# undistro/trivy

Hardware: AMD Instinct MI355X
Metric: GB/s secret-scanned (whole node) at 1/2/4/8 MI355X; findings bit-exact vs CPU (higher is better)
Workload: dtype u8

## Files before the change

### trivy_amd/csrc/engine.hip

```cpp
#include <chrono>
#include <condition_variable>
#include <mutex>
#include <hip/hip_runtime.h>

#include <algorithm>
#include <cstdlib>
#include <cstdio>
#include <cstring>
#include <string>
#include <pthread.h>

#include <thread>
#include <type_traits>

#include "engine.h"
#include "fetch.h"
#include "fetch_host.h"
#include "fetch_windows.h"
#include "xform.h"
#include "filter.h"

namespace tsg {

namespace {

constexpr int kScanThreads = 1024;
constexpr int kScanWaves = kScanThreads / 64;

#define HIP_OK(x)                                                   \
  do {                                                              \
    hipError_t e_ = (x);                                            \
    if (e_ != hipSuccess) {                                         \
      err_ = std::string(#x) + ": " + hipGetErrorString(e_);        \
      return false;                                                 \
    }                                                               \
  } while (0)


constexpr uint32_t kK0Run = 16;
struct ClearParams {
  uint32_t* flags;
  uint32_t* kw;
  uint64_t n_kw;
  uint32_t* counters;
  uint32_t* fs_ctr;
  uint32_t* skip_info;
};
__device__ __forceinline__ void clear_words(uint32_t* p, uint64_t n, uint64_t tid, uint64_t nthr) {
  const uint64_t n4 = n / 4;
  for (uint64_t i = tid; i < n4; i += nthr) reinterpret_cast<uint4*>(p)[i] = make_uint4(0, 0, 0, 0);
  if (tid < n % 4) p[4 * n4 + tid] = 0;
}
__global__ __launch_bounds__(256) void chunk_map_kernel(const uint64_t* __restrict__ off, uint32_t n_files,
                                                        uint64_t n_chunks, uint32_t* __restrict__ chunk_file,
                                                        ClearParams Z) {
  {
    const uint64_t tid = uint64_t(blockIdx.x) * blockDim.x + threadIdx.x, nthr = uint64_t(gridDim.x) * blockDim.x;
    clear_words(Z.flags, n_files, tid, nthr);
    clear_words(Z.kw, Z.n_kw, tid, nthr);
    if (tid < 16) {
      Z.counters[tid] = 0;
      if (Z.fs_ctr) Z.fs_ctr[tid] = 0;
      if (Z.skip_info) Z.skip_info[tid] = 0;
    }
  }
  const uint64_t n_runs = (n_chunks + kK0Run - 1) / kK0Run;
  for (uint64_t r = uint64_t(blockIdx.x) * blockDim.x + threadIdx.x; r < n_runs;
       r += uint64_t(gridDim.x) * blockDim.x) {
    const uint64_t c0 = r * kK0Run;
    uint64_t x = c0 * kChunk;
    uint32_t lo = 0, hi = n_files;
    while (hi - lo > 1) {
      const uint32_t mid = (lo + hi) >> 1;
      if (off[mid] <= x) lo = mid;
      else hi = mid;
    }
    uint32_t v[kK0Run];
    uint64_t fe = off[lo + 1];
#pragma unroll
    for (uint32_t i = 0; i < kK0Run; i++) {
      x = (c0 + i) * kChunk;
      while (x >= fe && lo + 1 < n_files) fe = off[++lo + 1];
      v[i] = lo;
    }
    if (c0 + kK0Run <= n_chunks) {
      uint4* d = reinterpret_cast<uint4*>(chunk_file + c0);
#pragma unroll
      for (uint32_t q = 0; q < kK0Run / 4; q++) d[q] = make_uint4(v[4 * q], v[4 * q + 1], v[4 * q + 2], v[4 * q + 3]);
    } else {
      for (uint32_t i = 0; c0 + i < n_chunks; i++) chunk_file[c0 + i] = v[i];
    }
  }
}

__device__ __forceinline__ uint4 load16(const uint8_t* p) { return *reinterpret_cast<const uint4*>(p); }

__device__ __forceinline__ void wave_sync() {
  __builtin_amdgcn_fence(__ATOMIC_RELEASE, "wavefront");
  __builtin_amdgcn_wave_barrier();
  __builtin_amdgcn_fence(__ATOMIC_ACQUIRE, "wavefront");
}

constexpr int kFLane = 64;
constexpr int kFBlocks = kFLane / 16;
constexpr int kFTile = 64 * kFLane;
constexpr int kFFlushAt = 128;
constexpr int kFQueue = kFFlushAt + 64;
constexpr int kFChunks = kFTile / 1024;
#ifndef TSG_K1_NLTILES
#define TSG_K1_NLTILES 16
#endif
constexpr int kFNlTiles = TSG_K1_NLTILES;
#ifndef TSG_K1_WGS
#define TSG_K1_WGS 2
#endif
constexpr int kFWgPerCu = TSG_K1_WGS;
#ifndef TSG_K1_GROUPQ
#define TSG_K1_GROUPQ 1
#endif
constexpr uint32_t kFGroup = 8;
#ifndef TSG_K1_READAHEAD
#define TSG_K1_READAHEAD 4
#endif
constexpr uint32_t kFReadAhead = TSG_K1_READAHEAD;
constexpr int kFWindow = 6;
constexpr int kFWords = 4;
constexpr uint32_t kFireBits = 0xFFF00000u;
constexpr uint32_t kNlBits = 0x8888u;
static_assert(kChunk % kFLane == 0 && kChunk / kFLane <= 64, "a newline chunk must be whole lane chunks");
static_assert(kFChunks * kChunk == kFTile && kFChunks == 4, "a tile's newline counts are one u64");

constexpr uint32_t kSkRuns = 0, kSkKept = 1, kSkTailKept = 2, kSkFiles = 3, kSkBytes = 4 ,
                   kSkWaveRuns = 6, kSkTiles = 7;

constexpr uint32_t kRunWords = 8;
__host__ __device__ inline uint64_t KeepWords(uint64_t n_tiles) {
  return ((n_tiles + 63) / 64 + kRunWords - 1) / kRunWords * kRunWords;
}

__global__ __launch_bounds__(256) void tile_keep_kernel(const uint64_t* __restrict__ off, uint32_t n_files,
                                                        const uint32_t* __restrict__ chunk_file,
                                                        const uint8_t* __restrict__ skip, uint64_t n_bytes,
                                                        uint64_t n_tiles, uint64_t* __restrict__ keep_bits,
                                                        uint32_t* __restrict__ info) {
  const uint32_t lane = threadIdx.x & 63u;
  const uint64_t stride = uint64_t(gridDim.x) * blockDim.x;
  const uint64_t n_padded = KeepWords(n_tiles) * 64;
  for (uint64_t base = uint64_t(blockIdx.x) * blockDim.x + (threadIdx.x & ~63u); base < n_padded; base += stride) {
    const uint64_t t = base + lane;
    bool keep = false;
    if (t < n_tiles) {
      const uint64_t ts = t * kFTile, te = ts + kFTile < n_bytes ? ts + kFTile : n_bytes;
      uint32_t f = chunk_file[t * kFChunks];
      for (;;) {
        const uint64_t fb = off[f], fe = off[f + 1];
        if (fe > fb && !skip[f]) {
          keep = true;
          break;
        }
        if (fe >= te || f + 1 >= n_files) break;
        f++;
      }
    }
    const uint64_t m = __ballot(keep);
    if (lane == 0) keep_bits[base / 64] = m;
  }
  constexpr uint32_t kStatBlocks = 64;
  if (blockIdx.x >= kStatBlocks) return;
  const uint64_t fstride = uint64_t(gridDim.x < kStatBlocks ? gridDim.x : kStatBlocks) * blockDim.x;
  uint32_t nf = 0;
  uint64_t nb = 0;
  for (uint64_t f = uint64_t(blockIdx.x) * blockDim.x + threadIdx.x; f < n_files; f += fstride)
    if (skip[f]) {
      nf++;
      nb += off[f + 1] - off[f];
    }
#pragma unroll
  for (int x = 1; x < 64; x <<= 1) {
    nf += __shfl_xor(nf, x);
    nb += __shfl_xor(nb, x);
  }
  if (lane == 0 && nf) {
    atomicAdd(&info[kSkFiles], nf);
    atomicAdd(reinterpret_cast<unsigned long long*>(&info[kSkBytes]), static_cast<unsigned long long>(nb));
  }
}

constexpr int kRunThreads = 1024;
__global__ __launch_bounds__(kRunThreads) void tile_runs_kernel(const uint64_t* __restrict__ keep_bits,
                                                                uint64_t n_tiles, uint2* __restrict__ runs,
                                                                uint32_t* __restrict__ info) {
  __shared__ uint32_t s_k[kRunThreads / 64], s_r[kRunThreads / 64];
  const uint32_t tid = threadIdx.x, lane = tid & 63u, wv = tid >> 6;
  const uint64_t n_words = KeepWords(n_tiles);
  const uint64_t per = ((n_words / kRunWords + kRunThreads - 1) / kRunThreads) * kRunWords;
  const uint64_t w0 = per * tid < n_words ? per * tid : n_words;
  const uint64_t w1 = w0 + per < n_words ? w0 + per : n_words;
  const uint64_t carry0 = w0 > 0 && w0 < n_words ? keep_bits[w0 - 1] >> 63 : 0;
  auto load_group = [&](uint64_t w, uint64_t* b) {
    const uint4* g = reinterpret_cast<const uint4*>(keep_bits + w);
#pragma unroll
    for (uint32_t q = 0; q < kRunWords / 2; q++) {
      const uint4 v = g[q];
      b[2 * q] = uint64_t(v.x) | (uint64_t(v.y) << 32);
      b[2 * q + 1] = uint64_t(v.z) | (uint64_t(v.w) << 32);
    }
  };
  uint32_t kept = 0, starts = 0;
  uint64_t carry = carry0;
  for (uint64_t w = w0; w < w1; w += kRunWords) {
    uint64_t g[kRunWords];
    load_group(w, g);
#pragma unroll
    for (uint32_t q = 0; q < kRunWords; q++) {
      const uint64_t b = g[q];
      kept += uint32_t(__popcll(b));
      starts += uint32_t(__popcll(b & ~((b << 1) | carry)));
      carry = b >> 63;
    }
  }
  uint32_t ik = kept, ir = starts;
#pragma unroll
  for (int x = 1; x < 64; x <<= 1) {
    const uint32_t a = __shfl_up(ik, x), b = __shfl_up(ir, x);
    if (lane >= uint32_t(x)) {
      ik += a;
      ir += b;
    }
  }
  if (lane == 63) {
    s_k[wv] = ik;
    s_r[wv] = ir;
  }
  __syncthreads();
  uint32_t bk = 0, br = 0;
  for (uint32_t q = 0; q < wv; q++) {
    bk += s_k[q];
    br += s_r[q];
  }
  uint32_t k = bk + ik - kept, r = br + ir - starts;
  carry = carry0;
  for (uint64_t w = w0; w < w1; w += kRunWords) {
    uint64_t g[kRunWords];
    load_group(w, g);
#pragma unroll
    for (uint32_t q = 0; q < kRunWords; q++) {
      const uint64_t b = g[q];
      for (uint64_t s = b & ~((b << 1) | carry); s; s &= s - 1) {
        const uint32_t bit = uint32_t(__builtin_ctzll(s));
        runs[r++] = make_uint2(uint32_t((w + q) * 64 + bit), k + uint32_t(__popcll(b & ((uint64_t(1) << bit) - 1))));
      }
      k += uint32_t(__popcll(b));
      carry = b >> 63;
    }
  }
  if (tid == kRunThreads - 1) {
    runs[r] = make_uint2(uint32_t(n_tiles), k);
    info[kSkRuns] = r;
    info[kSkKept] = k;
    info[kSkTailKept] = n_tiles ? uint32_t((keep_bits[(n_tiles - 1) / 64] >> ((n_tiles - 1) & 63)) & 1) : 0u;
    info[kSkTiles] = uint32_t(n_tiles);
  }
}

struct FilterParams {
  const uint8_t* arena;
  uint64_t n_bytes;
  const uint2* runs;
  uint32_t* run_info;
  const uint32_t* reach;
  uint32_t diag_mode;
  uint16_t* nl;
  uint32_t* recs;
  uint32_t rec_cap;
  uint32_t* counters;
};

__device__ __forceinline__ uint4 reach_read(const uint8_t* sb, uint32_t w, uint32_t k, uint32_t laneoff) {
  return *reinterpret_cast<const uint4*>(sb + __builtin_amdgcn_perm(w, laneoff, 0x0C0C0000u | ((4u + k) << 8)));
}

__device__ __forceinline__ void reach_apply(const uint4& m, uint32_t* st) {
  asm("v_lshl_or_b32 %0, %1, 4, %2" : "=v"(st[0]) : "v"(st[0]), "v"(m.x));
  asm("v_lshl_or_b32 %0, %1, 4, %2" : "=v"(st[1]) : "v"(st[1]), "v"(m.y));
  asm("v_lshl_or_b32 %0, %1, 4, %2" : "=v"(st[2]) : "v"(st[2]), "v"(m.z));
  asm("v_lshl_or_b32 %0, %1, 4, %2" : "=v"(st[3]) : "v"(st[3]), "v"(m.w));
}

__device__ __forceinline__ uint32_t nl_count4(uint32_t w) {
  const uint32_t a = ((w ^ 0x0A0A0A0Au) & 0x7F7F7F7Fu) + 0x7F7F7F7Fu;
  return __popc(~(a | w) & 0x80808080u);
}

__device__ __forceinline__ uint32_t word_of(uint4 v, uint32_t i) {
  return i < 2 ? (i == 0 ? v.x : v.y) : (i == 2 ? v.z : v.w);
}

__device__ __forceinline__ void load_reach_lds(uint8_t* s_reach, const uint32_t* reach, uint32_t copies, int tid,
                                               int nthreads) {
  for (uint32_t i = tid; i < 256 * copies; i += nthreads) {
    const uint32_t b = i / copies;
    reinterpret_cast<uint4*>(s_reach)[i] = reinterpret_cast<const uint4*>(reach)[b];
  }
}

template <bool kRuns>
__global__ __launch_bounds__(kScanThreads, 8) void filter_kernel(FilterParams P) {
  __shared__ __attribute__((aligned(16))) uint8_t s_reach[65536];
  __shared__ uint32_t s_queue[kScanWaves * kFQueue];
  __shared__ uint64_t s_nl[kScanWaves * kFNlTiles];
  const int tid = threadIdx.x;
  load_reach_lds(s_reach, P.reach, 16, tid, blockDim.x);
  __syncthreads();
  const uint32_t lane = tid & 63;
  const uint32_t wave = __builtin_amdgcn_readfirstlane(uint32_t(tid) >> 6);
  const uint32_t laneoff = (lane & 15) * 16;
  uint32_t* Q = s_queue + wave * kFQueue;
  uint64_t* NL = s_nl + wave * kFNlTiles;
  uint32_t nl_slots = 0;
  uint32_t qn = 0;
  const uint64_t n_tiles = (P.n_bytes + kFTile - 1) / kFTile;
  const uint64_t n_waves = uint64_t(gridDim.x) * kScanWaves;
  const uint64_t wid = uint64_t(blockIdx.x) * kScanWaves + wave;
  const uint2* __restrict__ RUNS = kRuns ? P.runs : nullptr;
  auto uni = [](uint32_t v) { return uint32_t(__builtin_amdgcn_readfirstlane(v)); };
  const uint64_t n_kept = RUNS ? uint64_t(uni(P.run_info[kSkKept])) : n_tiles;
  const bool tail_kept = RUNS ? uni(P.run_info[kSkTailKept]) != 0 : true;
  const uint64_t per = n_kept / n_waves, extra = n_kept % n_waves;
  const uint64_t k_begin = wid * per + (wid < extra ? wid : extra);
  const uint64_t k_end = k_begin + per + (wid < extra ? 1 : 0);
  uint32_t run = 0;
  uint64_t run_k1 = n_kept;
  uint64_t t_begin = k_begin;
  uint32_t runs_walked = 1;
  if (RUNS && k_begin < k_end) {
    uint32_t lo = 0, hi = uni(P.run_info[kSkRuns]);
    while (hi - lo > 1) {
      const uint32_t mid = (lo + hi) >> 1;
      if (uni(RUNS[mid].y) <= k_begin) lo = mid;
      else hi = mid;
    }
    run = lo;
    const uint2 r0 = RUNS[lo];
    t_begin = uint64_t(uni(r0.x)) + (k_begin - uni(r0.y));
    run_k1 = uni(RUNS[lo + 1].y);
  }
  uint4 bufA[kFBlocks], bufB[kFBlocks];
  uint32_t pre_x = 0, pre_y = 0;
  auto load_pre = [&](uint64_t tt) {
    const uint2 pv = *reinterpret_cast<const uint2*>(P.arena + tt * kFTile - 8);
    pre_x = __builtin_amdgcn_readfirstlane(pv.x);
    pre_y = __builtin_amdgcn_readfirstlane(pv.y);
  };
  if (k_begin < k_end && t_begin > 0) load_pre(t_begin);
  auto next_tile = [&](uint64_t k1, uint64_t tcur, bool* nr) -> uint64_t {
    if (k1 < run_k1) {
      *nr = false;
      return tcur + 1;
    }
    run++;
    runs_walked++;
    run_k1 = uni(RUNS[run + 1].y);
    *nr = true;
    return uni(RUNS[run].x);
  };
  auto load_tile = [&](uint4* dst, uint64_t tt) {
    const uint64_t b0 = tt * kFTile + uint64_t(lane) * kFLane;
    const uint8_t* lp = P.arena + (b0 < P.n_bytes ? b0 : 0);
#pragma unroll
    for (int j = 0; j < kFBlocks; j++) dst[j] = load16(lp + 16 * j);
  };
  auto flush = [&]() {
    uint32_t base = 0;
    if (lane == 0) base = atomicAdd(&P.counters[7], qn);
    base = __builtin_amdgcn_readfirstlane(base);
    for (uint32_t i = lane; i < qn; i += 64) {
      if (base + i < P.rec_cap) P.recs[base + i] = Q[i];
      else P.counters[8] = 1;
    }
    qn = 0;
  };
#if TSG_K1_GROUPQ
  uint32_t fl_acc = 0;
  uint32_t grp_n = 0;
  uint64_t grp_t0 = 0;
  auto compact = [&]() {
    const uint32_t cnt = __popc(fl_acc);
    uint32_t incl = cnt;
    incl += uint32_t(__builtin_amdgcn_update_dpp(0, int(incl), 0x111, 0xF, 0xF, true));
    incl += uint32_t(__builtin_amdgcn_update_dpp(0, int(incl), 0x112, 0xF, 0xF, true));
    incl += uint32_t(__builtin_amdgcn_update_dpp(0, int(incl), 0x114, 0xF, 0xF, true));
    incl += uint32_t(__builtin_amdgcn_update_dpp(0, int(incl), 0x118, 0xF, 0xF, true));
    incl += uint32_t(__builtin_amdgcn_update_dpp(0, int(incl), 0x142, 0xA, 0xF, false));
    incl += uint32_t(__builtin_amdgcn_update_dpp(0, int(incl), 0x143, 0xC, 0xF, false));
    const uint32_t total = __builtin_amdgcn_readlane(incl, 63);
    if (total) {
      if (qn + total > kFQueue) flush();
      const uint32_t rec0 = __builtin_amdgcn_readfirstlane(uint32_t(grp_t0 * (kFTile / 16))) + lane * kFBlocks;
      uint32_t m = fl_acc;
      if (total <= kFQueue) {
        uint32_t at = qn + incl - cnt;
        while (m) {
          const uint32_t b = uint32_t(__builtin_ctz(m));
          m &= m - 1;
          Q[at++] = rec0 + ((b >> 2) << 8) + (b & 3u);
        }
        qn += total;
      } else {
        uint32_t base = 0;
        if (lane == 0) base = atomicAdd(&P.counters[7], total);
        uint32_t at = __builtin_amdgcn_readfirstlane(base) + incl - cnt;
        while (m) {
          const uint32_t b = uint32_t(__builtin_ctz(m));
          m &= m - 1;
          if (at < P.rec_cap) P.recs[at] = rec0 + ((b >> 2) << 8) + (b & 3u);
          else P.counters[8] = 1;
          at++;
        }
      }
    }
    fl_acc = 0;
    grp_n = 0;
  };
#endif
  auto flush_nl = [&](uint64_t t_last) {
    wave_sync();
    uint32_t l = lane;
    asm volatile("" : "+v"(l));
    if (l < nl_slots) {
      const uint64_t tt = t_last - uint64_t(nl_slots - 1 - l);
      reinterpret_cast<uint64_t*>(P.nl)[tt] = NL[l];
    }
    nl_slots = 0;
  };
  auto tile = [&](uint4* cur, uint64_t tt, auto tail_tag) {
    constexpr bool kTail = decltype(tail_tag)::value;
    if (kTail) {
      const uint64_t b0 = tt * kFTile + uint64_t(lane) * kFLane;
#pragma unroll
      for (int j = 0; j < kFBlocks; j++) {
        const uint64_t p = b0 + 16 * j;
        uint32_t wd[4] = {cur[j].x, cur[j].y, cur[j].z, cur[j].w};
#pragma unroll
        for (int q = 0; q < 4; q++) {
          const uint64_t wp = p + 4 * q;
          if (wp >= P.n_bytes) wd[q] = 0;
          else if (wp + 4 > P.n_bytes) wd[q] &= (1u << (8 * (P.n_bytes - wp))) - 1u;
        }
        cur[j] = make_uint4(wd[0], wd[1], wd[2], wd[3]);
      }
    }
    const uint32_t p0 = uint32_t(__builtin_amdgcn_update_dpp(int(pre_x), int(cur[kFBlocks - 1].z), 0x138, 0xF, 0xF,
                                                             false));
    const uint32_t p1 = uint32_t(__builtin_amdgcn_update_dpp(int(pre_y), int(cur[kFBlocks - 1].w), 0x138, 0xF, 0xF,
                                                             false));
    pre_x = __builtin_amdgcn_readlane(cur[kFBlocks - 1].z, 63);
    pre_y = __builtin_amdgcn_readlane(cur[kFBlocks - 1].w, 63);
    uint32_t flagged = 0, nl = 0;
    if (P.diag_mode < 2) {
      uint32_t st[kFWords] = {~0u, ~0u, ~0u, ~0u};
      reach_apply(reach_read(s_reach, p0, 3, laneoff), st);
#pragma unroll
      for (uint32_t k = 0; k < 4; k++) reach_apply(reach_read(s_reach, p1, k, laneoff), st);
#pragma unroll
      for (int j = 0; j < kFBlocks; j++) {
        const uint32_t wd[4] = {cur[j].x, cur[j].y, cur[j].z, cur[j].w};
        uint32_t acc = ~0u;
#pragma unroll
        for (uint32_t g = 0; g < 16; g += kFReadAhead) {
          uint4 m[kFReadAhead];
#pragma unroll
          for (uint32_t q = 0; q < kFReadAhead; q++)
            m[q] = reach_read(s_reach, wd[(g + q) >> 2], (g + q) & 3, laneoff);
#pragma unroll
          for (uint32_t q = 0; q < kFReadAhead; q++) {
            const uint32_t k = g + q;
            reach_apply(m[q], st);
            if (k % 3 == 2 || k == 15) acc &= st[0] & st[1] & st[2] & st[3];
            if (k % 4 == 3) nl += __popc(~st[3] & kNlBits);
          }
        }
        flagged |= uint32_t((acc | ~kFireBits) != ~0u) << j;
      }
    } else {
#pragma unroll
      for (int j = 0; j < kFBlocks; j++)
        nl += nl_count4(cur[j].x) + nl_count4(cur[j].y) + nl_count4(cur[j].z) + nl_count4(cur[j].w);
    }
    {
    nl += uint32_t(__builtin_amdgcn_update_dpp(0, int(nl), 0x111, 0xF, 0xF, true));
    nl += uint32_t(__builtin_amdgcn_update_dpp(0, int(nl), 0x112, 0xF, 0xF, true));
    nl += uint32_t(__builtin_amdgcn_update_dpp(0, int(nl), 0x114, 0xF, 0xF, true));
    nl += uint32_t(__builtin_amdgcn_update_dpp(0, int(nl), 0x118, 0xF, 0xF, true));
    static_assert(kChunk / kFLane == 16, "one newline chunk per DPP row");
    static_assert(kFTile / 16 == 256, "a tile's records: 256 blocks");
    if ((lane & 15) == 15) reinterpret_cast<uint16_t*>(NL + nl_slots)[lane >> 4] = uint16_t(nl);
    if (++nl_slots == kFNlTiles) flush_nl(tt);
    }
#if TSG_K1_GROUPQ
    if (grp_n == 0) grp_t0 = tt;
    fl_acc |= flagged << (4 * grp_n);
    grp_n++;
#else
    const uint32_t rec0 = uint32_t(tt * (kFTile / 16)) + lane * kFBlocks;
#pragma unroll
    for (int j = 0; j < kFBlocks; j++) {
      const bool fj = (flagged >> j) & 1u;
      const uint64_t m = __ballot(fj);
      if (m) {
        if (qn + 64 > kFQueue) flush();
        const uint32_t below =
            __builtin_amdgcn_mbcnt_hi(uint32_t(m >> 32), __builtin_amdgcn_mbcnt_lo(uint32_t(m), 0u));
        if (fj) Q[qn + below] = rec0 + uint32_t(j);
        qn += uint32_t(__popcll(m));
      }
    }
#endif
  };
  auto flush_due = [&]() {
#if TSG_K1_GROUPQ
    if (grp_n == kFGroup) compact();
#endif
    if (qn >= kFFlushAt) flush();
  };
  using Full = std::false_type;
  if constexpr (!kRuns) {
    const uint64_t t_end = k_end;
    const uint64_t t_full = t_end < P.n_bytes / kFTile ? t_end : P.n_bytes / kFTile;
    uint64_t t = t_begin;
    if (t < t_full) load_tile(bufA, t);
    while (t < t_full) {
      flush_due();
      load_tile(bufB, t + 1 < t_full ? t + 1 : t);
      tile(bufA, t, Full());
      t++;
      if (t >= t_full) break;
      flush_due();
      load_tile(bufA, t + 1 < t_full ? t + 1 : t);
      tile(bufB, t, Full());
      t++;
    }
    if (t < t_end) {
      flush_due();
      load_tile(bufA, t);
      tile(bufA, t, std::true_type());
      t++;
    }
#if TSG_K1_GROUPQ
    if (grp_n) compact();
#endif
    if (qn) flush();
    if (nl_slots) flush_nl(t - 1);
    return;
  }
  const bool partial = (P.n_bytes % kFTile) != 0 && tail_kept;
  const uint64_t k_full = (partial && k_end == n_kept && k_end > k_begin) ? k_end - 1 : k_end;
  uint64_t k = k_begin, t = t_begin, t_prev = t_begin;
  bool nr_cur = false;
  auto run_boundary = [&]() {
#if TSG_K1_GROUPQ
    if (grp_n) compact();
#endif
    if (nl_slots) flush_nl(t_prev);
  };
  auto step = [&](uint4* cur, uint4* nxt) {
    if (nr_cur) run_boundary();
    flush_due();
    uint64_t tn = t;
    bool nr_n = false;
    if (k + 1 < k_end) tn = next_tile(k + 1, t, &nr_n);
    if (nr_cur) load_pre(t);
    load_tile(nxt, k + 1 < k_full ? tn : t);
    tile(cur, t, Full());
    t_prev = t;
    t = tn;
    nr_cur = nr_n;
    k++;
  };
  if (k < k_full) load_tile(bufA, t);
  while (k < k_full) {
    step(bufA, bufB);
    if (k >= k_full) break;
    step(bufB, bufA);
  }
  if (k < k_end) {
    if (nr_cur) run_boundary();
    flush_due();
    if (nr_cur) load_pre(t);
    load_tile(bufA, t);
    tile(bufA, t, std::true_type());
    t_prev = t;
    k++;
  }
#if TSG_K1_GROUPQ
  if (grp_n) compact();
#endif
  if (qn) flush();
  if (nl_slots) flush_nl(t_prev);
  if (RUNS && lane == 0 && k_begin < k_end) atomicMax(&P.run_info[kSkWaveRuns], runs_walked);
}

struct NfaParams {
  const uint8_t* arena;
  const uint64_t* off;
  uint32_t n_files;
  const uint16_t* nl;
  const AnchorInfo* anchors;
  const RuleGpu* rules;
  const uint32_t* rule_kw;
  const uint32_t* kwbits;
  uint32_t kw_words;
  const uint32_t* flags;
  const uint64_t* nfa;
  const uint32_t* hits;
  uint32_t hit_cap;
  uint32_t* counters;
  Candidate* cands;
  uint32_t cand_cap;
  const uint32_t* fullscan_rules;
  uint32_t n_fullscan_rules;
  uint32_t fs_chunk;
  uint32_t kw_fold;
  uint32_t diag;
  const uint8_t* skip;
};

__device__ __forceinline__ bool kw_bits_inexact(const NfaParams& P, uint32_t f) {
  return (P.flags[f] & 4u) && !(P.kw_fold && P.counters[10] == 0);
}



#ifndef TSG_C_THREADS
#define TSG_C_THREADS 512
#endif
constexpr int kCThreads = TSG_C_THREADS;
#ifndef TSG_C_THREADS_G
#define TSG_C_THREADS_G 256
#endif
constexpr int kCThreadsG = TSG_C_THREADS_G;
template <bool kLdsTabs>
constexpr int ConfirmThreads() { return kLdsTabs ? kCThreads : kCThreadsG; }

struct FoldSite {
  uint64_t x;
  uint32_t f;
  uint32_t len;
};

__device__ __forceinline__ uint32_t wave_slot(uint32_t* ctr) {
  const uint64_t m = __ballot(1);
  const uint32_t leader = uint32_t(__ffsll(static_cast<unsigned long long>(m)) - 1);
  const uint32_t rank = __builtin_amdgcn_mbcnt_hi(uint32_t(m >> 32), __builtin_amdgcn_mbcnt_lo(uint32_t(m), 0u));
  uint32_t base = 0;
  if (rank == 0) base = atomicAdd(ctr, uint32_t(__popcll(m)));
  base = __shfl(base, int(leader));
  return base + rank;
}

#ifndef TSG_C_HITS
#define TSG_C_HITS 96
#endif
constexpr uint32_t kCWaveHits = TSG_C_HITS;

constexpr uint32_t kHitAidBits = 24;
__device__ __forceinline__ uint32_t hit_aid_word(uint32_t aid, uint64_t end) {
  return aid | (uint32_t(end >> 32) << kHitAidBits);
}
__host__ __device__ __forceinline__ void hit_unpack(const uint32_t* h, uint32_t* f, uint64_t* end, uint32_t* aid) {
  *f = h[0];
  *end = uint64_t(h[1]) | (uint64_t(h[2] >> kHitAidBits) << 32);
  *aid = h[2] & ((1u << kHitAidBits) - 1u);
}

__device__ __forceinline__ void stage_hit(uint32_t* hbuf, uint32_t* hcnt, uint32_t* hits, uint32_t cap,
                                          uint32_t* counters, uint32_t f, uint64_t end, uint32_t aid) {
  const uint32_t k = atomicAdd(hcnt, 1u);
  if (k < kCWaveHits) {
    hbuf[3 * k + 0] = f;
    hbuf[3 * k + 1] = uint32_t(end);
    hbuf[3 * k + 2] = hit_aid_word(aid, end);
    return;
  }
  const uint32_t g = atomicAdd(&counters[0], 1u);
  if (g < cap) {
    hits[3ull * g + 0] = f;
    hits[3ull * g + 1] = uint32_t(end);
    hits[3ull * g + 2] = hit_aid_word(aid, end);
  } else {
    counters[3] = 1;
  }
}

__device__ __forceinline__ void flush_staged(uint32_t* hbuf, uint32_t* hcnt, uint32_t* hits, uint32_t cap,
                                             uint32_t* counters, uint32_t lane) {
  wave_sync();
  const uint32_t n_all = __builtin_amdgcn_readfirstlane(*hcnt);
  const uint32_t n = n_all < kCWaveHits ? n_all : kCWaveHits;
  if (n) {
    uint32_t base = 0;
    if (lane == 0) base = atomicAdd(&counters[0], n);
    base = __builtin_amdgcn_readfirstlane(base);
    for (uint32_t i = lane; i < n; i += 64) {
      if (base + i < cap) {
        hits[3ull * (base + i) + 0] = hbuf[3 * i + 0];
        hits[3ull * (base + i) + 1] = hbuf[3 * i + 1];
        hits[3ull * (base + i) + 2] = hbuf[3 * i + 2];
      } else {
        counters[3] = 1;
      }
    }
  }
  wave_sync();
  if (lane == 0) *hcnt = 0;
  wave_sync();
}

__device__ __forceinline__ void put_hit(uint32_t* hits, uint32_t cap, uint32_t* counters, uint32_t f, uint64_t end,
                                        uint32_t aid) {
  const uint32_t g = wave_slot(&counters[0]);
  if (g < cap) {
    hits[3ull * g + 0] = f;
    hits[3ull * g + 1] = uint32_t(end);
    hits[3ull * g + 2] = hit_aid_word(aid, end);
  } else {
    counters[3] = 1;
  }
}
__device__ __forceinline__ bool follow_lut_pass(const FollowLut& L, const uint32_t* X, int64_t avail) {
  const uint32_t n0 = L.n[0], n1 = L.n[1];
  if (n0 == 0) return true;
  const int64_t span0 = int64_t(L.hi[0]) + n0, span1 = n1 ? int64_t(L.hi[1]) + n1 : 0;
  const int64_t lim = avail < (span0 > span1 ? span0 : span1) ? avail : (span0 > span1 ? span0 : span1);
  uint32_t nonascii = 0;
#pragma unroll
  for (int j = 0; j < 13; j++) {
    const int64_t v = lim - 4 * j;
    const uint32_t vm = v >= 4 ? ~0u : (v <= 0 ? 0u : (1u << (8 * uint32_t(v))) - 1u);
    nonascii |= X[j] & vm;
  }
  if (nonascii & 0x80808080u) return true;
  uint32_t t[4], h[2];
  __builtin_memcpy(t, L.lo_tab, 16);
  __builtin_memcpy(h, L.hi_tab, 8);
  uint32_t M[13];
#pragma unroll
  for (int j = 0; j < 13; j++) {
    const uint32_t lo = X[j] & 0x0F0F0F0Fu, hi = (X[j] >> 4) & 0x07070707u;
    const uint32_t sel = lo & 0x07070707u;
    const uint32_t a0 = __builtin_amdgcn_perm(t[1], t[0], sel), a1 = __builtin_amdgcn_perm(t[3], t[2], sel);
    const uint32_t m8 = ((lo >> 3) & 0x01010101u) * 0xFFu;
    M[j] = ((a0 & ~m8) | (a1 & m8)) & __builtin_amdgcn_perm(h[1], h[0], hi);
  }
  auto interval = [&](int r, uint32_t n) -> uint64_t {
    int64_t a = L.lo[r], b = L.hi[r];
    if (avail - int64_t(n) < b) b = avail - int64_t(n);
    if (b < a) return 0;
    const uint64_t upto = b >= 63 ? ~uint64_t(0) : (uint64_t(1) << (b + 1)) - 1;
    return upto & ~((uint64_t(1) << a) - 1);
  };
  const uint64_t R0 = interval(0, n0), R1 = n1 ? interval(1, n1) : 0;
  uint32_t f0 = 0, f1 = 0;
#pragma unroll
  for (int j = 0; j < 12; j++) {
    const uint32_t y1 = __builtin_amdgcn_alignbyte(M[j + 1], M[j], 1);
    const uint32_t y2 = __builtin_amdgcn_alignbyte(M[j + 1], M[j], 2);
    const uint32_t y3 = __builtin_amdgcn_alignbyte(M[j + 1], M[j], 3);
    const uint32_t Z = M[j] & (y1 >> 1) & (y2 >> 2) & (y3 >> 3);
    const uint32_t s0 = ((uint32_t(R0 >> (4 * j)) & 0xFu) * 0x00204081u) & 0x01010101u;
    const uint32_t s1 = ((uint32_t(R1 >> (4 * j)) & 0xFu) * 0x00204081u) & 0x01010101u;
    f0 |= Z & s0;
    f1 |= Z & (s1 << 4);
  }
  return f0 != 0 && (n1 == 0 || f1 != 0);
}

__device__ __forceinline__ void follow_words(const uint32_t* w, uint32_t s, uint32_t* X) {
  uint32_t R[14];
#pragma unroll
  for (int j = 0; j < 14; j++) R[j] = w[j];
#pragma unroll
  for (int j = 0; j < 13; j++) X[j] = __builtin_amdgcn_alignbyte(R[j + 1], R[j], s & 3);
}

#ifndef TSG_C_WIN
#define TSG_C_WIN 48
#endif
constexpr int kCWin = TSG_C_WIN;

struct ConfirmParams {
  const uint8_t* arena;
  uint64_t n_bytes;
  const uint64_t* off;
  const uint32_t* chunk_file;
  const uint16_t* nl;
  const uint32_t* reach;
  const void* tabs;
  uint32_t tabs_bytes, t_bucket_off, t_bucket_items, t_items, t_item_ids, t_item_cls, t_classes;
  const AnchorInfo* anchors;
  const RuleGpu* rules;
  const uint64_t* nfa;
  const uint32_t* recs;
  uint32_t rec_cap;
  uint32_t* flags;
  uint32_t* counters;
  uint32_t* hits;
  uint32_t hit_cap;
  FoldSite* folds;
  uint32_t fold_cap;
  uint32_t diag;
  uint32_t* kwbits;
  uint32_t kw_words;
  const uint64_t* core;
  const uint32_t* group_items;
  const uint32_t* bucket_groups;
  uint32_t* item_diag;
  uint32_t t_luts;
  uint32_t t_cmap, t_ccore, t_gitems, t_bgroups, n_cls;
  uint32_t t_hkeys, t_hitems, hash_bits, hash_buckets;
  uint32_t n_classes_lds;
  const uint8_t* wins;
};

constexpr int kNfaReject = 0, kNfaAccept = 1, kNfaUndecided = 2;
template <int W>
__device__ int nfa_run_abs(const uint8_t* __restrict arena, uint64_t fs, int64_t len, int64_t start, int64_t inj_hi,
                           const uint64_t* __restrict tab, int64_t max_steps) {
  uint64_t O[W], Lp[W], F[W], D[W];
#pragma unroll
  for (int w = 0; w < W; w++) {
    O[w] = tab[w];
    Lp[w] = tab[W + w];
    F[w] = tab[2 * W + w];
    D[w] = 0;
  }
  const uint64_t* B = tab + 3 * W;
  uint4 buf = make_uint4(0, 0, 0, 0);
  uint64_t buf_at = ~uint64_t(0);
  const int64_t stop = len - start > max_steps ? start + max_steps : len;
  for (int64_t pos = start; pos < stop; pos++) {
    const uint64_t abs = fs + uint64_t(pos);
    if ((abs & ~uint64_t(15)) != buf_at) {
      buf_at = abs & ~uint64_t(15);
      buf = load16(arena + buf_at);
    }
    const uint32_t b = (word_of(buf, uint32_t(abs >> 2) & 3) >> ((abs & 3) * 8)) & 0xFFu;
    uint64_t carry = pos <= inj_hi ? 1 : 0;
    uint64_t T[W];
#pragma unroll
    for (int w = 0; w < W; w++) {
      T[w] = (D[w] << 1) | carry | (D[w] & Lp[w]);
      carry = D[w] >> 63;
    }
    uint64_t c = 0;
#pragma unroll
    for (int w = 0; w < W; w++) {
      uint64_t x = T[w] & O[w];
      uint64_t s1 = O[w] + x;
      uint64_t c1 = s1 < O[w];
      uint64_t s2 = s1 + c;
      uint64_t c2 = s2 < s1;
      T[w] |= s2 ^ O[w];
      c = c1 | c2;
    }
    const uint64_t* Bb = B + size_t(b) * W;
    const bool keep = (b & 0xC0u) == 0x80u;
    uint64_t acc = 0, alive = 0;
#pragma unroll
    for (int w = 0; w < W; w++) {
      uint64_t nd = (T[w] & Bb[w]) | (keep ? D[w] : 0);
      D[w] = nd;
      acc |= nd & F[w];
      alive |= nd;
    }
    if (acc) return kNfaAccept;
    if (!alive && pos >= inj_hi) return kNfaReject;
  }
  return stop < len ? kNfaUndecided : kNfaReject;
}

__device__ int nfa_dispatch_abs(int words, const uint8_t* arena, uint64_t fs, int64_t len, int64_t start,
                                int64_t inj_hi, const uint64_t* tab, int64_t max_steps = INT64_MAX) {
  switch (words) {
    case 1: return nfa_run_abs<1>(arena, fs, len, start, inj_hi, tab, max_steps);
    case 2: return nfa_run_abs<2>(arena, fs, len, start, inj_hi, tab, max_steps);
    case 3: return nfa_run_abs<3>(arena, fs, len, start, inj_hi, tab, max_steps);
    default: return nfa_run_abs<4>(arena, fs, len, start, inj_hi, tab, max_steps);
  }
}

__device__ __forceinline__ void put_candidate(Candidate* cands, uint32_t cap, uint32_t* counters, uint32_t f,
// ... 3172 lines not shown
```

Baseline: 2611.

## Carry NFA boundary state across lanes instead of re-scanning predecessor bytes

Each lane used to start its shift-and state by replaying the previous lane's last five bytes through the reach table, which cost extra LDS reads per tile. Lanes now start from a zero state. The first-block states at steps 2 and 5 are packed, and the end-of-lane state is passed to the neighbouring lane by DPP with a per-wave readlane carry, so that matches crossing a lane boundary are still detected. Tile ranges and loop bounds are also forced scalar via readfirstlane so that address and control math stays on the SALU. This adds packing and permute work per tile and relies on the combined boundary check matching the old per-byte semantics exactly.

```diff
diff --git a/trivy_amd/csrc/engine.hip b/trivy_amd/csrc/engine.hip
--- a/trivy_amd/csrc/engine.hip
+++ b/trivy_amd/csrc/engine.hip
@@ -127,6 +127,7 @@
 constexpr int kFWords = 4;
 constexpr uint32_t kFireBits = 0xFFF00000u;
 constexpr uint32_t kNlBits = 0x8888u;
+constexpr uint32_t kFirePacked = 0xFFF0FFF0u;
 static_assert(kChunk % kFLane == 0 && kChunk / kFLane <= 64, "a newline chunk must be whole lane chunks");
 static_assert(kFChunks * kChunk == kFTile && kFChunks == 4, "a tile's newline counts are one u64");
 
@@ -292,6 +293,10 @@
   return __popc(~(a | w) & 0x80808080u);
 }
 
+__device__ __forceinline__ uint32_t pack_hi16(uint32_t hi, uint32_t lo) {
+  return __builtin_amdgcn_perm(hi, lo, 0x07060302u);
+}
+
 __device__ __forceinline__ uint32_t word_of(uint4 v, uint32_t i) {
   return i < 2 ? (i == 0 ? v.x : v.y) : (i == 2 ? v.z : v.w);
 }
@@ -326,9 +331,10 @@
   auto uni = [](uint32_t v) { return uint32_t(__builtin_amdgcn_readfirstlane(v)); };
   const uint64_t n_kept = RUNS ? uint64_t(uni(P.run_info[kSkKept])) : n_tiles;
   const bool tail_kept = RUNS ? uni(P.run_info[kSkTailKept]) != 0 : true;
+  auto uni64 = [&](uint64_t v) { return (uint64_t(uni(uint32_t(v >> 32))) << 32) | uni(uint32_t(v)); };
   const uint64_t per = n_kept / n_waves, extra = n_kept % n_waves;
-  const uint64_t k_begin = wid * per + (wid < extra ? wid : extra);
-  const uint64_t k_end = k_begin + per + (wid < extra ? 1 : 0);
+  const uint64_t k_begin = uni64(wid * per + (wid < extra ? wid : extra));
+  const uint64_t k_end = uni64(k_begin + per + (wid < extra ? 1 : 0));
   uint32_t run = 0;
   uint64_t run_k1 = n_kept;
   uint64_t t_begin = k_begin;
@@ -346,13 +352,26 @@
     run_k1 = uni(RUNS[lo + 1].y);
   }
   uint4 bufA[kFBlocks], bufB[kFBlocks];
-  uint32_t pre_x = 0, pre_y = 0;
-  auto load_pre = [&](uint64_t tt) {
-    const uint2 pv = *reinterpret_cast<const uint2*>(P.arena + tt * kFTile - 8);
-    pre_x = __builtin_amdgcn_readfirstlane(pv.x);
-    pre_y = __builtin_amdgcn_readfirstlane(pv.y);
+  uint32_t carry[4] = {0, 0, 0, 0};
+  auto boundary_words = [](const uint32_t* st, uint32_t* q) {
+    q[0] = pack_hi16(st[1] << 12, st[0] << 12);
+    q[1] = pack_hi16(st[3] << 12, st[2] << 12);
+    q[2] = __builtin_amdgcn_perm(st[1], st[0], 0x040C000Cu);
+    q[3] = __builtin_amdgcn_perm(st[3], st[2], 0x040C000Cu);
   };
-  if (k_begin < k_end && t_begin > 0) load_pre(t_begin);
+  auto load_carry = [&](uint64_t tt) {
+    uint2 pv = make_uint2(0, 0);
+    if (tt > 0) pv = *reinterpret_cast<const uint2*>(P.arena + tt * kFTile - 8);
+    uint32_t st[kFWords] = {~0u, ~0u, ~0u, ~0u};
+    reach_apply(reach_read(s_reach, pv.x, 3, laneoff), st);
+#pragma unroll
+    for (uint32_t k = 0; k < 4; k++) reach_apply(reach_read(s_reach, pv.y, k, laneoff), st);
+    uint32_t q[4];
+    boundary_words(st, q);
+#pragma unroll
+    for (int i = 0; i < 4; i++) carry[i] = __builtin_amdgcn_readfirstlane(q[i]);
+  };
+  if (k_begin < k_end) load_carry(t_begin);
   auto next_tile = [&](uint64_t k1, uint64_t tcur, bool* nr) -> uint64_t {
     if (k1 < run_k1) {
       *nr = false;
@@ -365,7 +384,9 @@
     return uni(RUNS[run].x);
   };
   auto load_tile = [&](uint4* dst, uint64_t tt) {
-    const uint64_t b0 = tt * kFTile + uint64_t(lane) * kFLane;
+    uint32_t l = lane;
+    asm volatile("" : "+v"(l));
+    const uint64_t b0 = tt * kFTile + uint64_t(l) * kFLane;
     const uint8_t* lp = P.arena + (b0 < P.n_bytes ? b0 : 0);
 #pragma unroll
     for (int j = 0; j < kFBlocks; j++) dst[j] = load16(lp + 16 * j);
@@ -450,18 +471,10 @@
         cur[j] = make_uint4(wd[0], wd[1], wd[2], wd[3]);
       }
     }
-    const uint32_t p0 = uint32_t(__builtin_amdgcn_update_dpp(int(pre_x), int(cur[kFBlocks - 1].z), 0x138, 0xF, 0xF,
-                                                             false));
-    const uint32_t p1 = uint32_t(__builtin_amdgcn_update_dpp(int(pre_y), int(cur[kFBlocks - 1].w), 0x138, 0xF, 0xF,
-                                                             false));
-    pre_x = __builtin_amdgcn_readlane(cur[kFBlocks - 1].z, 63);
-    pre_y = __builtin_amdgcn_readlane(cur[kFBlocks - 1].w, 63);
     uint32_t flagged = 0, nl = 0;
     if (P.diag_mode < 2) {
-      uint32_t st[kFWords] = {~0u, ~0u, ~0u, ~0u};
-      reach_apply(reach_read(s_reach, p0, 3, laneoff), st);
-#pragma unroll
-      for (uint32_t k = 0; k < 4; k++) reach_apply(reach_read(s_reach, p1, k, laneoff), st);
+      uint32_t st[kFWords] = {0u, 0u, 0u, 0u};
+      uint32_t pk[4] = {0u, 0u, 0u, 0u};
 #pragma unroll
       for (int j = 0; j < kFBlocks; j++) {
         const uint32_t wd[4] = {cur[j].x, cur[j].y, cur[j].z, cur[j].w};
@@ -476,12 +489,25 @@
           for (uint32_t q = 0; q < kFReadAhead; q++) {
             const uint32_t k = g + q;
             reach_apply(m[q], st);
-            if (k % 3 == 2 || k == 15) acc &= st[0] & st[1] & st[2] & st[3];
+            if (j == 0 && (k == 2 || k == 5)) {
+              pk[k == 2 ? 0 : 2] = pack_hi16(st[1], st[0]);
+              pk[k == 2 ? 1 : 3] = pack_hi16(st[3], st[2]);
+            } else if (k % 3 == 2 || k == 15) {
+              acc &= st[0] & st[1] & st[2] & st[3];
+            }
             if (k % 4 == 3) nl += __popc(~st[3] & kNlBits);
           }
         }
         flagged |= uint32_t((acc | ~kFireBits) != ~0u) << j;
       }
+      uint32_t q[4], z = ~0u;
+      boundary_words(st, q);
+#pragma unroll
+      for (int i = 0; i < 4; i++) {
+        z &= pk[i] | uint32_t(__builtin_amdgcn_update_dpp(int(carry[i]), int(q[i]), 0x138, 0xF, 0xF, false));
+        carry[i] = __builtin_amdgcn_readlane(q[i], 63);
+      }
+      flagged |= uint32_t((z | ~kFirePacked) != ~0u);
     } else {
 #pragma unroll
       for (int j = 0; j < kFBlocks; j++)
@@ -494,7 +520,11 @@
     nl += uint32_t(__builtin_amdgcn_update_dpp(0, int(nl), 0x118, 0xF, 0xF, true));
     static_assert(kChunk / kFLane == 16, "one newline chunk per DPP row");
     static_assert(kFTile / 16 == 256, "a tile's records: 256 blocks");
-    if ((lane & 15) == 15) reinterpret_cast<uint16_t*>(NL + nl_slots)[lane >> 4] = uint16_t(nl);
+    {
+      uint32_t l = lane;
+      asm volatile("" : "+v"(l));
+      if ((l & 15) == 15) reinterpret_cast<uint16_t*>(NL + nl_slots)[l >> 4] = uint16_t(nl);
+    }
     if (++nl_slots == kFNlTiles) flush_nl(tt);
     }
 #if TSG_K1_GROUPQ
@@ -554,7 +584,7 @@
     return;
   }
   const bool partial = (P.n_bytes % kFTile) != 0 && tail_kept;
-  const uint64_t k_full = (partial && k_end == n_kept && k_end > k_begin) ? k_end - 1 : k_end;
+  const uint64_t k_full = uni64((partial && k_end == n_kept && k_end > k_begin) ? k_end - 1 : k_end);
   uint64_t k = k_begin, t = t_begin, t_prev = t_begin;
   bool nr_cur = false;
   auto run_boundary = [&]() {
@@ -569,7 +599,7 @@
     uint64_t tn = t;
     bool nr_n = false;
     if (k + 1 < k_end) tn = next_tile(k + 1, t, &nr_n);
-    if (nr_cur) load_pre(t);
+    if (nr_cur) load_carry(t);
     load_tile(nxt, k + 1 < k_full ? tn : t);
     tile(cur, t, Full());
     t_prev = t;
@@ -586,7 +616,7 @@
   if (k < k_end) {
     if (nr_cur) run_boundary();
     flush_due();
-    if (nr_cur) load_pre(t);
+    if (nr_cur) load_carry(t);
     load_tile(bufA, t);
     tile(bufA, t, std::true_type());
     t_prev = t;
```

Result: no change. 2664, median of 6 (+2.0%).
